# lorenlugosch/end-to-end-SLU

Hardware: AMD Instinct MI355X
Metric: utterances/sec (train step, 3 s @16 kHz, B=64) (higher is better)
Workload: dtype f32 (trainable stages: exact fp32 MFMA; convolutions and GRU contractions of FROZEN stages: bf16x3 = every fp32 operand split EXACTLY into 3 bf16 terms (3 x 8 = 24 significand bits, fp32's exponent range), 6 bf16 MFMA products per fp32 product (only terms below 2^-24 |a b| dropped), fp32 accumulatio; 1 GPU; experiments/no_unfreezing.cfg SLU train step (frozen SincNet/conv/biGRU encoder in train mode + intent biGRU trained): fwd + 3-slot CE + bwd + grad all-reduce + Adam; batch_per_gpu=64, global_batch=64, samples_per_utterance=48000, parallelism=dp1, encoder_lookahead_batches=20

## Files before the change

### end-to-end-slu_amd/csrc/slu_gru_bf16.hip

```cpp
#include "slu_bf16.h"
#include <type_traits>

namespace slu {

__device__ __forceinline__ float bf_sigmoid(float x) {
  return __builtin_amdgcn_rcpf(1.0f + __builtin_amdgcn_exp2f(-1.4426950408889634f * x));
}
__device__ __forceinline__ float bf_tanh(float x) {
  return 1.0f - 2.0f * __builtin_amdgcn_rcpf(1.0f + __builtin_amdgcn_exp2f(2.8853900817779268f * x));
}

__device__ __forceinline__ void lds_barrier() { asm volatile("s_waitcnt lgkmcnt(0)\n\ts_barrier" ::: "memory"); }

__device__ __forceinline__ float mul_rnd(float a, float b) {
#pragma clang fp contract(off)
  return a * b;
}
__device__ __forceinline__ float add_rnd(float a, float b) {
#pragma clang fp contract(off)
  return a + b;
}

struct GruBfParams {
  const float* gx;
  const unsigned short* xp; long long x_plane;
  const uint4* wih; const float* b_ih;
  const float* w_hh[2];
  const float* b_hh[2];
  float* out;
  float* reserve;
  unsigned short* planes; long long plane;
  const unsigned* keep;
  float keep_scale;
  int T, B, D;
};

template <int H, int NS, int KI, int EPI>
struct GruLds {
  static constexpr int ROWB = H * 2;
  static constexpr int GXROW = 3 * H + 8;
  static constexpr int OROW = H + 4;
  static constexpr int PROWB = H * 2 + 16;
  static constexpr int HBUF = 2 * NS * 16 * ROWB;
  static constexpr int BIAS = KI > 0 ? 2 * 3 * H * 4 : 0;
  static constexpr int GXS = KI > 0 ? 0 : 2 * 16 * GXROW * 4;
  static constexpr int OST = EPI == 1 ? 2 * NS * 16 * PROWB : 2 * 16 * OROW * 4;
  static constexpr int BYTES = HBUF + BIAS + GXS + OST;
};

template <int H, int NS, int KI, int EPI, bool REV>
__device__ __forceinline__ void gru_bf_fwd_body(const GruBfParams& p) {
  constexpr int NW = H / 16;
  constexpr int KC = H / 32;
  constexpr int SLOTS = H / 8;
  constexpr bool BIAS_LDS = KI > 0;
  typedef Split<NS> SP;
  typedef GruLds<H, NS, KI, EPI> LD;
  constexpr int ROWB = LD::ROWB, GXROW = LD::GXROW, OROW = LD::OROW, PROWB = LD::PROWB;
  extern __shared__ __attribute__((aligned(16))) unsigned char smem[];
  unsigned char* const hbuf = smem;
  float* const bias_s = reinterpret_cast<float*>(smem + LD::HBUF);
  float* const gxs = reinterpret_cast<float*>(smem + LD::HBUF + LD::BIAS);
  unsigned char* const ost = smem + LD::HBUF + LD::BIAS + LD::GXS;
  const int tid = threadIdx.x, lane = tid & 63;
  const int w = __builtin_amdgcn_readfirstlane(tid >> 6);
  const int i = lane & 15, kg = lane >> 4;
  constexpr int dir = REV ? 1 : 0;
  const int b0 = blockIdx.x * 16;
  const int u0 = w * 16 + kg * 4;
  const int T = p.T, B = p.B, D = p.D;
  const int seq = b0 + i;
  const int seqc = seq < B ? seq : B - 1;

  if constexpr (NS == 2) f16_denorm_flush();

  uint4 wb[3][KC][NS];
  {
    const float* __restrict__ W = p.w_hh[dir];
#pragma unroll
    for (int g = 0; g < 3; ++g)
#pragma unroll
      for (int c = 0; c < KC; ++c) {
        const float* src = W + (size_t)(g * H + w * 16 + i) * H + c * 32 + kg * 8;
        const float4 lo = *reinterpret_cast<const float4*>(src), hi = *reinterpret_cast<const float4*>(src + 4);
        const float v[8] = {lo.x, lo.y, lo.z, lo.w, hi.x, hi.y, hi.z, hi.w};
        unsigned short s[8][NS];
#pragma unroll
        for (int e = 0; e < 8; ++e) split_terms<NS>(v[e], s[e]);
#pragma unroll
        for (int pl = 0; pl < NS; ++pl) {
          uint4 o;
          o.x = s[0][pl] | ((unsigned)s[1][pl] << 16); o.y = s[2][pl] | ((unsigned)s[3][pl] << 16);
          o.z = s[4][pl] | ((unsigned)s[5][pl] << 16); o.w = s[6][pl] | ((unsigned)s[7][pl] << 16);
          wb[g][c][pl] = o;
        }
      }
  }
  float bh[3][4];
  if constexpr (BIAS_LDS) {
    for (int x = tid; x < 3 * H; x += H * 4) {
      bias_s[x] = p.b_hh[dir][x];
      bias_s[3 * H + x] = p.b_ih[(size_t)dir * 3 * H + x];
    }
  } else {
#pragma unroll
    for (int g = 0; g < 3; ++g) {
      const float4 v = *reinterpret_cast<const float4*>(p.b_hh[dir] + g * H + u0);
      bh[g][0] = v.x; bh[g][1] = v.y; bh[g][2] = v.z; bh[g][3] = v.w;
    }
  }
  constexpr int KIA = KI > 0 ? KI : 1;
  uint4 wi[3][KIA][NS];
  if constexpr (KI > 0) {
    const int NTI = p.D * 3 * NW;
#pragma unroll
    for (int g = 0; g < 3; ++g)
#pragma unroll
      for (int c = 0; c < KI; ++c)
#pragma unroll
        for (int pl = 0; pl < NS; ++pl)
          wi[g][c][pl] = p.wih[(size_t)pl * KI * NTI * 64 + ((size_t)c * NTI + dir * 3 * NW + g * NW + w) * 64 + lane];
  }
  auto xproj = [&](const uint4 (&xa)[KIA][NS], float (&o)[3][4]) {
    f32x4 ax[SP::NACC][3];
#pragma unroll
    for (int a = 0; a < SP::NACC; ++a)
#pragma unroll
      for (int g = 0; g < 3; ++g) ax[a][g] = f32x4{0.f, 0.f, 0.f, 0.f};
#pragma unroll
    for (int c = 0; c < KIA; ++c)
#pragma unroll
      for (int q = 0; q < SP::NPAIR; ++q)
#pragma unroll
        for (int g = 0; g < 3; ++g)
          ax[SP::ACC(q)][g] = mfma_split<NS>(wi[g][c][SP::PB(q)], xa[c][SP::PA(q)], ax[SP::ACC(q)][g]);
#pragma unroll
    for (int g = 0; g < 3; ++g) {
      const f32x4 v = split_result<NS>(ax[0][g], ax[SP::NACC - 1][g]);
      const float4 bi = *reinterpret_cast<const float4*>(&bias_s[BIAS_LDS ? 3 * H + g * H + u0 : 0]);
      o[g][0] = v[0] + bi.x; o[g][1] = v[1] + bi.y; o[g][2] = v[2] + bi.z; o[g][3] = v[3] + bi.w;
    }
  };
  auto xload = [&](int t_, uint4 (&xa)[KIA][NS]) {
    const unsigned short* base = p.xp + ((size_t)t_ * B + seqc) * (32 * KIA) + kg * 8;
#pragma unroll
    for (int c = 0; c < KIA; ++c)
#pragma unroll
      for (int pl = 0; pl < NS; ++pl)
        xa[c][pl] = *reinterpret_cast<const uint4*>(base + (size_t)pl * p.x_plane + c * 32);
  };

  constexpr int RW = 16 / NW;
  constexpr int GLR = 3 * H / 4;
  auto gx_g = [&](int j) { const int f = j * 64 + lane; return min(b0 + RW * w + f / GLR, B - 1) * D * 3 * H + dir * 3 * H + (f % GLR) * 4; };
  auto gx_s = [&](int j) { const int f = j * 64 + lane; return (RW * w + f / GLR) * GXROW + (f % GLR) * 4; };
  const int gx_g0 = gx_g(0), gx_g1 = gx_g(1), gx_g2 = gx_g(2);
  const int gx_s0 = gx_s(0), gx_s1 = gx_s(1), gx_s2 = gx_s(2);
  const size_t gx_ts = (size_t)B * D * 3 * H, out_ts = (size_t)B * D * H;
#define SLU_GX_REQUEST(t_, a, b, c)                                                         \
  do {                                                                                      \
    const float* gp__ = p.gx + (size_t)(t_) * gx_ts;                                        \
    a = *reinterpret_cast<const float4*>(gp__ + gx_g0);                                     \
    b = *reinterpret_cast<const float4*>(gp__ + gx_g1);                                     \
    c = *reinterpret_cast<const float4*>(gp__ + gx_g2);                                     \
  } while (0)
#define SLU_GX_STAGE(buf, a, b, c)                                                          \
  do {                                                                                      \
    float* gs__ = gxs + (buf) * (16 * GXROW);                                               \
    *reinterpret_cast<float4*>(gs__ + gx_s0) = a;                                           \
    *reinterpret_cast<float4*>(gs__ + gx_s1) = b;                                           \
    *reinterpret_cast<float4*>(gs__ + gx_s2) = c;                                           \
  } while (0)
  const int orow = RW * w + lane / (H / 4), oc16 = lane % (H / 4);
  const bool orow_ok = b0 + orow < B;
  const int o_goff = (b0 + orow) * D * H + dir * H + oc16 * 4;

  int a_off[KC];
#pragma unroll
  for (int c = 0; c < KC; ++c) a_off[c] = i * ROWB + (((c * 4 + kg) ^ i) & (SLOTS - 1)) * 16;
  const int h_off = i * ROWB + ((((u0 >> 3) ^ i) & (SLOTS - 1)) * 16) + (u0 & 7) * 2;
  const int gs_off = i * GXROW + u0;
  const int os_off = i * OROW + u0;
  const int ps_off = i * PROWB + u0 * 2;
  const int kw_off = seqc * ((D * H) >> 5) + ((dir * H + u0) >> 5);
  const int kw_sh = (dir * H + u0) & 31;
  const size_t kw_ts = (size_t)B * ((D * H) >> 5);
  const bool drop = EPI > 0 && p.keep != nullptr;

  for (int x = tid; x < 2 * NS * 16 * ROWB / 4; x += H * 4) reinterpret_cast<unsigned*>(hbuf)[x] = 0u;
  float hprev[4] = {0.f, 0.f, 0.f, 0.f};
  float gcur[3][4];
  unsigned kcur = 0;
  {
    const int t0 = dir ? T - 1 : 0;
    if constexpr (KI > 0) {
      __syncthreads();
      uint4 xa0[KIA][NS];
      xload(t0, xa0);
      xproj(xa0, gcur);
    } else {
      float4 ga, gb, gc;
      SLU_GX_REQUEST(t0, ga, gb, gc);
      SLU_GX_STAGE(0, ga, gb, gc);
    }
    if (drop) kcur = p.keep[(size_t)t0 * kw_ts + kw_off];
  }
  float held[4] = {0.f, 0.f, 0.f, 0.f};
  int pend_t = -1;
  int pend_buf = 0;
  auto flush = [&]() {
    if (pend_t < 0) return;
    if constexpr (EPI == 1) {
      constexpr int LPR = H / 8;
      constexpr int NCH = NS * 16 * LPR / 64;
      for (int c = w; c < NCH; c += NW) {
        const int f = c * 64 + lane, pl = f / (16 * LPR), r = (f / LPR) % 16, c16 = f % LPR;
        if (b0 + r < B) {
          const uint4 v = *reinterpret_cast<const uint4*>(ost + ((pend_buf * NS + pl) * 16 + r) * PROWB + c16 * 16);
          *reinterpret_cast<uint4*>(p.planes + (size_t)pl * p.plane + (size_t)pend_t * out_ts + (b0 + r) * D * H + dir * H + c16 * 8) = v;
        }
      }
    } else {
      if (orow_ok) {
        const float4 v = *reinterpret_cast<const float4*>(reinterpret_cast<const float*>(ost) + (pend_buf * 16 + orow) * OROW + oc16 * 4);
        *reinterpret_cast<float4*>(p.out + (size_t)pend_t * out_ts + o_goff) = v;
      }
    }
  };
  __syncthreads();
  __builtin_amdgcn_s_waitcnt(0x0F70);

  auto step = [&](auto cur_c, const int s) {
    constexpr int cur = decltype(cur_c)::value;
    const int t = dir ? T - 1 - s : s;
    const int tn = (s + 1 < T) ? (dir ? t - 1 : t + 1) : t;

    if constexpr (BIAS_LDS) {
#pragma unroll
      for (int g = 0; g < 3; ++g) {
        const float4 v = *reinterpret_cast<const float4*>(&bias_s[g * H + u0]);
        bh[g][0] = v.x; bh[g][1] = v.y; bh[g][2] = v.z; bh[g][3] = v.w;
      }
    }
    if constexpr (KI == 0) {
#pragma unroll
      for (int g = 0; g < 3; ++g) {
        const float4 v = *reinterpret_cast<const float4*>(gxs + cur * (16 * GXROW) + gs_off + g * H);
        gcur[g][0] = v.x; gcur[g][1] = v.y; gcur[g][2] = v.z; gcur[g][3] = v.w;
      }
    }
    f32x4 accs[SP::NACC][3];
#pragma unroll
    for (int a = 0; a < SP::NACC; ++a)
#pragma unroll
      for (int g = 0; g < 3; ++g) accs[a][g] = f32x4{0.f, 0.f, 0.f, 0.f};
    float gn[4];
#pragma unroll
    for (int r = 0; r < 4; ++r) {
      accs[0][0][r] = gcur[0][r] + bh[0][r];
      accs[0][1][r] = gcur[1][r] + bh[1][r];
      accs[0][2][r] = bh[2][r];
      gn[r] = gcur[2][r];
    }
    const unsigned kbits = kcur >> kw_sh;

    float gnext[3][4];
    float4 gl0 = make_float4(0.f, 0.f, 0.f, 0.f), gl1 = gl0, gl2 = gl0;
    uint4 xan[KIA][NS];
    if constexpr (KI > 0) xload(tn, xan);
    else SLU_GX_REQUEST(tn, gl0, gl1, gl2);
    unsigned knext = 0;
    if (drop) knext = p.keep[(size_t)tn * kw_ts + kw_off];
    flush();

    const unsigned char* hc = hbuf + cur * (NS * 16 * ROWB);
    float hn[4];
#pragma unroll
    for (int c = 0; c < KC; ++c) {
      uint4 fa[NS];
#pragma unroll
      for (int pl = 0; pl < NS; ++pl) fa[pl] = *reinterpret_cast<const uint4*>(hc + pl * (16 * ROWB) + a_off[c]);
#pragma unroll
      for (int q = 0; q < SP::NPAIR; ++q)
#pragma unroll
        for (int g = 0; g < 3; ++g)
          accs[SP::ACC(q)][g] = mfma_split<NS>(wb[g][c][SP::PB(q)], fa[SP::PA(q)], accs[SP::ACC(q)][g]);
    }
    f32x4 acc[3];
#pragma unroll
    for (int g = 0; g < 3; ++g) acc[g] = split_result<NS>(accs[0][g], accs[SP::NACC - 1][g]);

#pragma unroll
    for (int r = 0; r < 4; ++r) {
      const float rr = bf_sigmoid(acc[0][r]);
      const float zz = bf_sigmoid(acc[1][r]);
      const float nn = bf_tanh(gn[r] + rr * acc[2][r]);
      hn[r] = nn + zz * (hprev[r] - nn);
    }
    {
      unsigned char* __restrict__ hnext = hbuf + (cur ^ 1) * (NS * 16 * ROWB);
      if constexpr (NS == 2) {
        unsigned hi01, lo01, hi23, lo23;
        split_f16x2_pair_flush(hn[0], hn[1], hi01, lo01);
        split_f16x2_pair_flush(hn[2], hn[3], hi23, lo23);
        *reinterpret_cast<uint2*>(hnext + h_off) = make_uint2(hi01, hi23);
        *reinterpret_cast<uint2*>(hnext + 16 * ROWB + h_off) = make_uint2(lo01, lo23);
      } else if constexpr (NS == 3) {
        unsigned w01[3], w23[3];
        split_bf16x3_pair(hn[0], hn[1], w01);
        split_bf16x3_pair(hn[2], hn[3], w23);
#pragma unroll
        for (int pl = 0; pl < 3; ++pl)
          *reinterpret_cast<uint2*>(hnext + pl * (16 * ROWB) + h_off) = make_uint2(w01[pl], w23[pl]);
      } else {
        unsigned short sp[4][NS];
#pragma unroll
        for (int r = 0; r < 4; ++r) split_terms<NS>(hn[r], sp[r]);
#pragma unroll
        for (int pl = 0; pl < NS; ++pl)
          *reinterpret_cast<uint2*>(hnext + pl * (16 * ROWB) + h_off) =
              make_uint2(sp[0][pl] | ((unsigned)sp[1][pl] << 16), sp[2][pl] | ((unsigned)sp[3][pl] << 16));
      }
    }
    if constexpr (EPI == 0) {
      *reinterpret_cast<float4*>(reinterpret_cast<float*>(ost) + cur * (16 * OROW) + os_off) = make_float4(hn[0], hn[1], hn[2], hn[3]);
      pend_t = t; pend_buf = cur;
    } else {
      float m[4];
#pragma unroll
      for (int r = 0; r < 4; ++r)
        m[r] = drop ? mul_rnd(hn[r], ((kbits >> r) & 1u) ? p.keep_scale : 0.0f) : hn[r];
      const bool even = dir ? (t & 1) == 0 : cur == 0;
      const bool single = even && t == T - 1;
      const bool emit = dir ? even : (!even || single);
      pend_t = -1;
      if (!emit) {
#pragma unroll
        for (int r = 0; r < 4; ++r) held[r] = dir ? m[r] : add_rnd(0.0f, m[r]);
      } else {
        float v[4];
#pragma unroll
        for (int r = 0; r < 4; ++r) {
          const float first = dir ? add_rnd(0.0f, m[r]) : held[r];
          const float second = dir ? held[r] : m[r];
          v[r] = mul_rnd(add_rnd(first, second), 0.5f);
        }
        if (single) {
          asm volatile("" ::: "memory");
#pragma unroll
          for (int r = 0; r < 4; ++r) v[r] = add_rnd(0.0f, m[r]);
        }
        pend_t = t >> 1; pend_buf = cur;
        if constexpr (EPI == 2) {
          *reinterpret_cast<float4*>(reinterpret_cast<float*>(ost) + cur * (16 * OROW) + os_off) = make_float4(v[0], v[1], v[2], v[3]);
        } else if constexpr (NS == 2) {
          unsigned hi01, lo01, hi23, lo23;
          split_f16x2_pair_flush(v[0], v[1], hi01, lo01);
          split_f16x2_pair_flush(v[2], v[3], hi23, lo23);
          *reinterpret_cast<uint2*>(ost + ((cur * NS + 0) * 16) * PROWB + ps_off) = make_uint2(hi01, hi23);
          *reinterpret_cast<uint2*>(ost + ((cur * NS + 1) * 16) * PROWB + ps_off) = make_uint2(lo01, lo23);
        } else if constexpr (NS == 3) {
          unsigned w01[3], w23[3];
          split_bf16x3_pair(v[0], v[1], w01);
          split_bf16x3_pair(v[2], v[3], w23);
#pragma unroll
          for (int pl = 0; pl < 3; ++pl)
            *reinterpret_cast<uint2*>(ost + ((cur * NS + pl) * 16) * PROWB + ps_off) = make_uint2(w01[pl], w23[pl]);
        } else {
          unsigned short sp[4][NS];
#pragma unroll
          for (int r = 0; r < 4; ++r) split_terms<NS>(v[r], sp[r]);
#pragma unroll
          for (int pl = 0; pl < NS; ++pl)
            *reinterpret_cast<uint2*>(ost + ((cur * NS + pl) * 16) * PROWB + ps_off) =
                make_uint2(sp[0][pl] | ((unsigned)sp[1][pl] << 16), sp[2][pl] | ((unsigned)sp[3][pl] << 16));
        }
      }
    }
    if constexpr (KI > 0) {
      xproj(xan, gnext);
#pragma unroll
      for (int g = 0; g < 3; ++g)
#pragma unroll
        for (int r = 0; r < 4; ++r) gcur[g][r] = gnext[g][r];
    } else {
      SLU_GX_STAGE(cur ^ 1, gl0, gl1, gl2);
    }
#pragma unroll
    for (int r = 0; r < 4; ++r) hprev[r] = hn[r];
    kcur = knext;
    lds_barrier();
  };
  {
    int s = 0;
    for (; s + 1 < T; s += 2) {
      step(std::integral_constant<int, 0>{}, s);
      step(std::integral_constant<int, 1>{}, s + 1);
    }
    if (s < T) step(std::integral_constant<int, 0>{}, s);
  }
  flush();
#undef SLU_GX_REQUEST
#undef SLU_GX_STAGE
}

template <int H, int NS, int KI, int EPI>
__global__ void __launch_bounds__(H * 4)
gru_bf_fwd_kernel(const GruBfParams p) {
  if (blockIdx.y) gru_bf_fwd_body<H, NS, KI, EPI, true>(p);
  else gru_bf_fwd_body<H, NS, KI, EPI, false>(p);
}

template <int H, int NS, int EPI>
struct Gru2Lds {
  static constexpr int ROWB = H * 2;
  static constexpr int OROW = H + 4;
  static constexpr int PROWB = H * 2 + 16;
  static constexpr int HB = NS * 16 * ROWB;
  static constexpr int GXB = 16 * 3 * H * 4;
  static constexpr int KBB = 16 * (H / 32) * 4;
  static constexpr int OSB = EPI == 1 ? NS * 16 * PROWB : 16 * OROW * 4;
  static constexpr int HBUF = 0;
  static constexpr int GXR = HBUF + 2 * HB;
  static constexpr int KBR = GXR + 3 * GXB;
  static constexpr int BIAS = KBR + 3 * KBB;
  static constexpr int OST = BIAS + 3 * H * 4;
  static constexpr int HP = OST + 2 * OSB;
  static constexpr int HELD = HP + 2 * 16 * H * 4;
  static constexpr int BYTES = HELD + (EPI > 0 ? 2 * 16 * H * 4 : 0);
};

__device__ __forceinline__ void dma_b128(const void* base, unsigned voff, unsigned lds_addr) {
  asm volatile("s_mov_b32 m0, %2\n\ts_nop 0\n\tglobal_load_lds_dwordx4 %0, %1" :: "v"(voff), "s"(base), "s"(lds_addr) : "memory");
}
__device__ __forceinline__ void dma_b32(const void* base, unsigned voff, unsigned lds_addr) {
  asm volatile("s_mov_b32 m0, %2\n\ts_nop 0\n\tglobal_load_lds_dword %0, %1" :: "v"(voff), "s"(base), "s"(lds_addr) : "memory");
}

template <int H, int NS, int EPI>
__global__ void __launch_bounds__(H * 4)
gru_bf2_fwd_kernel(const GruBfParams p) {
  static_assert(H == 128, "two-tile recurrence: H = 128 (8 waves = two per SIMD, one keep-word DMA per chunk)");
  constexpr int NW = H / 16, KC = H / 32, SLOTS = H / 8;
  typedef Split<NS> SP;
  typedef Gru2Lds<H, NS, EPI> LD;
  constexpr int ROWB = LD::ROWB, OROW = LD::OROW, PROWB = LD::PROWB;
  constexpr int PCS = 3 * H / 4;
  extern __shared__ __attribute__((aligned(16))) unsigned char smem[];
  typedef __attribute__((address_space(3))) void* lptr_t;
  const unsigned lds0 = (unsigned)(size_t)(lptr_t)smem;
  float* const bias_s = reinterpret_cast<float*>(smem + LD::BIAS);
  const int tid = threadIdx.x, lane = tid & 63;
  const int w = __builtin_amdgcn_readfirstlane(tid >> 6);
  const int i = lane & 15, kg = lane >> 4;
  const int dir = blockIdx.y;
  const int b0 = blockIdx.x * 32;
  const int u0 = w * 16 + kg * 4;
  const int T = p.T, B = p.B, D = p.D;

  if constexpr (NS == 2) f16_denorm_flush();

  uint4 wb[3][KC][NS];
  {
    const float* __restrict__ W = p.w_hh[dir];
#pragma unroll
    for (int g = 0; g < 3; ++g)
#pragma unroll
      for (int c = 0; c < KC; ++c) {
        const float* src = W + (size_t)(g * H + w * 16 + i) * H + c * 32 + kg * 8;
        const float4 lo = *reinterpret_cast<const float4*>(src), hi = *reinterpret_cast<const float4*>(src + 4);
        const float v[8] = {lo.x, lo.y, lo.z, lo.w, hi.x, hi.y, hi.z, hi.w};
        unsigned short s[8][NS];
#pragma unroll
        for (int e = 0; e < 8; ++e) split_terms<NS>(v[e], s[e]);
#pragma unroll
        for (int pl = 0; pl < NS; ++pl) {
          uint4 o;
          o.x = s[0][pl] | ((unsigned)s[1][pl] << 16); o.y = s[2][pl] | ((unsigned)s[3][pl] << 16);
          o.z = s[4][pl] | ((unsigned)s[5][pl] << 16); o.w = s[6][pl] | ((unsigned)s[7][pl] << 16);
          wb[g][c][pl] = o;
        }
      }
  }
  for (int x = tid; x < 3 * H; x += H * 4) bias_s[x] = p.b_hh[dir][x];
  for (int x = tid; x < 2 * LD::HB / 4; x += H * 4) reinterpret_cast<unsigned*>(smem + LD::HBUF)[x] = 0u;
  __syncthreads();

  const bool drop = EPI > 0 && p.keep != nullptr;
  unsigned gv[2][3];
#pragma unroll
  for (int x = 0; x < 2; ++x)
#pragma unroll
    for (int j = 0; j < 3; ++j) {
      const int P = (3 * w + j) * 64 + lane, row = P / PCS, q = P % PCS;
      gv[x][j] = (unsigned)((min(b0 + 16 * x + row, B - 1) * D * 3 * H + dir * 3 * H) * 4 + (q ^ (row & 15)) * 16);
    }
  unsigned kv[2];
  const int KW = (D * H) >> 5;
#pragma unroll
  for (int x = 0; x < 2; ++x)
    kv[x] = drop ? (unsigned)((min(b0 + 16 * x + (lane >> 2), B - 1) * KW + dir * (H >> 5) + (lane & 3)) * 4) : (unsigned)(lane * 4);
  const void* const kbase = drop ? (const void*)p.keep : (const void*)p.gx;
  const size_t gx_ts = (size_t)B * D * 3 * H * 4, kw_ts = drop ? (size_t)B * KW * 4 : 0, out_ts = (size_t)B * D * H;
  const unsigned gx_m0 = lds0 + LD::GXR + 3 * w * 1024, kb_m0 = lds0 + LD::KBR;
  auto dma_chunk = [&](int x, int t_, int slot) {
    const char* gb = reinterpret_cast<const char*>(p.gx) + (size_t)t_ * gx_ts;
    const unsigned m = gx_m0 + slot * LD::GXB;
    const unsigned v0 = x ? gv[1][0] : gv[0][0], v1 = x ? gv[1][1] : gv[0][1], v2 = x ? gv[1][2] : gv[0][2];
    dma_b128(gb, v0, m);
    dma_b128(gb, v1, m + 1024);
    dma_b128(gb, v2, m + 2048);
    dma_b32(reinterpret_cast<const char*>(kbase) + (size_t)t_ * kw_ts, x ? kv[1] : kv[0], kb_m0 + slot * LD::KBB);
  };

  const int a_off0 = i * ROWB + ((kg ^ i) & (SLOTS - 1)) * 16;
  const int h_off = i * ROWB + ((((u0 >> 3) ^ i) & (SLOTS - 1)) * 16) + (u0 & 7) * 2;
  const int gs_off0 = (i * PCS + ((u0 >> 2) ^ i)) * 16;
  const int hp_off = (i * H + u0) * 4;
  const int kb_off = (i * (H >> 5) + (u0 >> 5)) * 4;
  const int kb_sh = u0 & 31;
  const int os_off = i * OROW + u0;
  const int ps_off = i * PROWB + u0 * 2;
  const int orow = (16 / NW) * w + lane / (H / 4), oc16 = lane % (H / 4);

  f32x4 accs[2][SP::NACC][3];
  float gn[2][4];
  unsigned kb[2] = {0u, 0u};
  int pend[2] = {-1, -1};
#pragma unroll
  for (int x = 0; x < 2; ++x) {
#pragma unroll
    for (int r = 0; r < 4; ++r) gn[x][r] = 0.f;
    *reinterpret_cast<float4*>(smem + LD::HP + x * (16 * H * 4) + hp_off) = make_float4(0.f, 0.f, 0.f, 0.f);
    if constexpr (EPI > 0) *reinterpret_cast<float4*>(smem + LD::HELD + x * (16 * H * 4) + hp_off) = make_float4(0.f, 0.f, 0.f, 0.f);
  }
#pragma unroll
  for (int x = 0; x < 2; ++x)
#pragma unroll
    for (int a = 0; a < SP::NACC; ++a)
#pragma unroll
      for (int g = 0; g < 3; ++g) accs[x][a][g] = f32x4{0.f, 0.f, 0.f, 0.f};

#define SLU_G2_M(X, slot)                                                                                              \
// ... 147 lines not shown
  dma_chunk(0, tt(0), 0);
  dma_chunk(1, tt(0), 1);
  asm volatile("s_waitcnt vmcnt(0)" ::: "memory");
  __syncthreads();

  int sl = 0;
  SLU_G2_PHASE(0, true, false, 0, tt(1));
  for (int s = 0; s + 1 < T; ++s) {
    SLU_G2_PHASE(1, true, true, tt(s), tt(s + 1));
    SLU_G2_PHASE(0, true, true, tt(s), tt(s + 2));
  }
  SLU_G2_PHASE(1, true, true, tt(T - 1), tt(T - 1));
  SLU_G2_PHASE(0, false, true, tt(T - 1), tt(T - 1));
  SLU_G2_FLUSH(1);
  asm volatile("s_waitcnt vmcnt(0)" ::: "memory");
#undef SLU_G2_PHASE
#undef SLU_G2_FLUSH
#undef SLU_G2_G
#undef SLU_G2_M
}

template <int H, int NS>
__global__ void __launch_bounds__(H * 4)
gru_bf_fwd_rs_kernel(const GruBfParams p) {
  constexpr int NW = H / 16, KC = H / 32, ROWB = H * 2, SLOTS = H / 8;
  typedef Split<NS> SP;
  __shared__ __attribute__((aligned(16))) unsigned char hbuf[2][NS][16 * ROWB];
  const int tid = threadIdx.x, lane = tid & 63;
  const int w = __builtin_amdgcn_readfirstlane(tid >> 6);
  const int i = lane & 15, kg = lane >> 4;
  const int dir = blockIdx.y;
  const int b0 = blockIdx.x * 16;
  const int j = w * 16 + i;
  const int T = p.T, B = p.B, D = p.D;

  uint4 wb[3][KC][NS];
  {
    const float* __restrict__ W = p.w_hh[dir];
#pragma unroll
    for (int g = 0; g < 3; ++g)
#pragma unroll
      for (int c = 0; c < KC; ++c) {
        const float* src = W + (size_t)(g * H + j) * H + c * 32 + kg * 8;
        const float4 lo = *reinterpret_cast<const float4*>(src), hi = *reinterpret_cast<const float4*>(src + 4);
        const float v[8] = {lo.x, lo.y, lo.z, lo.w, hi.x, hi.y, hi.z, hi.w};
        unsigned short s[8][NS];
#pragma unroll
        for (int e = 0; e < 8; ++e) split_terms<NS>(v[e], s[e]);
#pragma unroll
        for (int pl = 0; pl < NS; ++pl) {
          uint4 o;
          o.x = s[0][pl] | ((unsigned)s[1][pl] << 16); o.y = s[2][pl] | ((unsigned)s[3][pl] << 16);
          o.z = s[4][pl] | ((unsigned)s[5][pl] << 16); o.w = s[6][pl] | ((unsigned)s[7][pl] << 16);
          wb[g][c][pl] = o;
        }
      }
  }
  const float bhr = p.b_hh[dir][j], bhz = p.b_hh[dir][H + j], bhn = p.b_hh[dir][2 * H + j];
  for (int x = tid; x < 2 * NS * 16 * ROWB / 4; x += H * 4) reinterpret_cast<unsigned*>(&hbuf[0][0][0])[x] = 0u;
  float hprev[4] = {0.f, 0.f, 0.f, 0.f};
  int g_off[4], o_off[4];
#pragma unroll
  for (int r = 0; r < 4; ++r) {
    const int b = b0 + 4 * kg + r;
    g_off[r] = (b < B ? b : 0) * D * 3 * H;
    o_off[r] = b < B ? b * D * H : -1;
  }
  const size_t gx_ts = (size_t)B * D * 3 * H, out_ts = (size_t)B * D * H;
  const float* __restrict__ gxd = p.gx + (size_t)dir * 3 * H + j;
  float* __restrict__ outd = p.out + (size_t)dir * H + j;
  int a_off[KC];
#pragma unroll
  for (int c = 0; c < KC; ++c) a_off[c] = i * ROWB + (((c * 4 + kg) ^ i) & (SLOTS - 1)) * 16;
  int h_off[4];
#pragma unroll
  for (int r = 0; r < 4; ++r) {
    const int row = 4 * kg + r;
    h_off[r] = row * ROWB + ((((j >> 3) ^ row) & (SLOTS - 1)) * 16) + (j & 7) * 2;
  }
  float gr[4], gz[4], gn[4];
  {
    const int t0 = dir ? T - 1 : 0;
#pragma unroll
    for (int r = 0; r < 4; ++r) {
      const float* g = gxd + (size_t)t0 * gx_ts + g_off[r];
      gr[r] = g[0]; gz[r] = g[H]; gn[r] = g[2 * H];
    }
  }
  __syncthreads();

  for (int s = 0; s < T; ++s) {
    const int t = dir ? T - 1 - s : s;
    const int cur = s & 1;
    float ngr[4], ngz[4], ngn[4];
    const int tn = (s + 1 < T) ? (dir ? t - 1 : t + 1) : t;
#pragma unroll
    for (int r = 0; r < 4; ++r) {
      const float* g = gxd + (size_t)tn * gx_ts + g_off[r];
      ngr[r] = g[0]; ngz[r] = g[H]; ngn[r] = g[2 * H];
    }
    f32x4 accs[SP::NACC][3];
#pragma unroll
    for (int a = 0; a < SP::NACC; ++a)
#pragma unroll
      for (int g = 0; g < 3; ++g) accs[a][g] = f32x4{0.f, 0.f, 0.f, 0.f};
#pragma unroll
    for (int c = 0; c < KC; ++c) {
      uint4 fa[NS];
#pragma unroll
      for (int pl = 0; pl < NS; ++pl) fa[pl] = *reinterpret_cast<const uint4*>(&hbuf[cur][pl][a_off[c]]);
#pragma unroll
      for (int q = 0; q < SP::NPAIR; ++q)
#pragma unroll
        for (int g = 0; g < 3; ++g)
          accs[SP::ACC(q)][g] = mfma_split<NS>(fa[SP::PA(q)], wb[g][c][SP::PB(q)], accs[SP::ACC(q)][g]);
    }
    f32x4 acc[3];
#pragma unroll
    for (int g = 0; g < 3; ++g) acc[g] = split_result<NS>(accs[0][g], accs[SP::NACC - 1][g]);

    float hn[4], rr[4], zz[4], nn[4], qq[4];
#pragma unroll
    for (int r = 0; r < 4; ++r) {
      rr[r] = bf_sigmoid(gr[r] + (acc[0][r] + bhr));
      zz[r] = bf_sigmoid(gz[r] + (acc[1][r] + bhz));
      qq[r] = acc[2][r] + bhn;
      nn[r] = bf_tanh(gn[r] + rr[r] * qq[r]);
      hn[r] = (1.0f - zz[r]) * nn[r] + zz[r] * hprev[r];
    }
    {
      float4* __restrict__ rs = reinterpret_cast<float4*>(
          p.reserve + ((((size_t)dir * T + t) * gridDim.x + blockIdx.x) * NW + w) * (5 * 256)) + lane;
      rs[0 * 64] = make_float4(rr[0], rr[1], rr[2], rr[3]);
      rs[1 * 64] = make_float4(zz[0], zz[1], zz[2], zz[3]);
      rs[2 * 64] = make_float4(nn[0], nn[1], nn[2], nn[3]);
      rs[3 * 64] = make_float4(qq[0], qq[1], qq[2], qq[3]);
      rs[4 * 64] = make_float4(hprev[0], hprev[1], hprev[2], hprev[3]);
    }
    unsigned char* __restrict__ hnext = &hbuf[cur ^ 1][0][0];
#pragma unroll
    for (int r = 0; r < 4; ++r) {
      unsigned short sp[NS];
      split_terms<NS>(hn[r], sp);
#pragma unroll
      for (int pl = 0; pl < NS; ++pl) *reinterpret_cast<unsigned short*>(hnext + pl * (16 * ROWB) + h_off[r]) = sp[pl];
      if (o_off[r] >= 0) outd[(size_t)t * out_ts + o_off[r]] = hn[r];
    }
#pragma unroll
    for (int r = 0; r < 4; ++r) { hprev[r] = hn[r]; gr[r] = ngr[r]; gz[r] = ngz[r]; gn[r] = ngn[r]; }
    __syncthreads();
  }
}

template <int H, int NS, int KI, int EPI>
static void gru_bf_launch(dim3 grid, hipStream_t st, const GruBfParams& p) {
  constexpr int lds = GruLds<H, NS, KI, EPI>::BYTES;
  static bool raised = false;
  if (lds > 64 * 1024 && !raised) {
    (void)hipFuncSetAttribute((const void*)gru_bf_fwd_kernel<H, NS, KI, EPI>, hipFuncAttributeMaxDynamicSharedMemorySize, lds);
    raised = true;
  }
  hipLaunchKernelGGL((gru_bf_fwd_kernel<H, NS, KI, EPI>), grid, dim3(H * 4), lds, st, p);
}

template <int H, int NS, int EPI>
static void gru_bf2_launch(hipStream_t st, const GruBfParams& p) {
  constexpr int lds = Gru2Lds<H, NS, EPI>::BYTES;
  static bool raised = false;
  if (lds > 64 * 1024 && !raised) {
    (void)hipFuncSetAttribute((const void*)gru_bf2_fwd_kernel<H, NS, EPI>, hipFuncAttributeMaxDynamicSharedMemorySize, lds);
    raised = true;
  }
  hipLaunchKernelGGL((gru_bf2_fwd_kernel<H, NS, EPI>), dim3((unsigned)cdiv(p.B, 32), (unsigned)p.D), dim3(H * 4), lds, st, p);
}

template <int H, int EPI>
static int gru_bf_dispatch(int nsplit, int ki, int seq_tiles, dim3 grid, hipStream_t st, const GruBfParams& p) {
  if (seq_tiles == 2) {
    if constexpr (H == 128) {
      if (nsplit == 3) gru_bf2_launch<128, 3, EPI>(st, p);
      else if (nsplit == 2) gru_bf2_launch<128, 2, EPI>(st, p);
      else gru_bf2_launch<128, 1, EPI>(st, p);
    }
    SLU_CHECK_LAUNCH("gru_bf2_fwd_kernel");
    return SLU_OK;
  }
  if (ki > 0) {
    if constexpr (H == 128) {
      if (nsplit == 3) {
        if (ki == 1) gru_bf_launch<128, 3, 1, EPI>(grid, st, p); else gru_bf_launch<128, 3, 2, EPI>(grid, st, p);
      } else {
        if (ki == 1) gru_bf_launch<128, 2, 1, EPI>(grid, st, p); else gru_bf_launch<128, 2, 2, EPI>(grid, st, p);
      }
    }
  } else if (nsplit == 3) {
    gru_bf_launch<H, 3, 0, EPI>(grid, st, p);
  } else if (nsplit == 2) {
    gru_bf_launch<H, 2, 0, EPI>(grid, st, p);
  } else {
    gru_bf_launch<H, 1, 0, EPI>(grid, st, p);
  }
  SLU_CHECK_LAUNCH("gru_bf_fwd_kernel");
  return SLU_OK;
}

}

using namespace slu;

static int gru_bf_common(const char* who, GruBfParams& p, const float* gx, const float* w_hh_fwd, const float* w_hh_rev,
                         const float* b_hh_fwd, const float* b_hh_rev, const void* x_planes, int64_t x_plane_stride,
                         int64_t K, const void* w_ih_packed, const float* b_ih, int64_t T, int64_t B, int64_t H, int64_t D,
                         int nsplit, bool has_reserve, int seq_tiles) {
  SLU_REQUIRE((gx || x_planes) && w_hh_fwd && b_hh_fwd, "%s: null pointer", who);
  SLU_REQUIRE(seq_tiles >= 0 && seq_tiles <= 2, "%s: seq_tiles must be 0 / 1 (one 16-sequence tile per workgroup) or 2", who);
  if (seq_tiles == 2 && !(H == 128 && gx && !x_planes && !has_reserve && B * D * 3 * H < (1LL << 30)))
    SLU_FAIL(SLU_ERR_UNSUPPORTED, "%s: two sequence tiles per workgroup are instantiated for H = 128, gx input (no fused "
             "projection), no reserve, B * D * 3H < 2^30 (got H %lld, B %lld)", who, (long long)H, (long long)B);
  const bool fused = x_planes != nullptr;
  if (fused) {
    SLU_REQUIRE(!gx && w_ih_packed && b_ih && !has_reserve, "%s: the fused input projection takes x_planes, "
                "w_ih_packed and b_ih instead of gx, and no reserve (frozen layers only)", who);
    if (!((nsplit == 2 || nsplit == 3) && H == 128 && K >= 1 && K <= 64))
      SLU_FAIL(SLU_ERR_UNSUPPORTED, "%s: the fused input projection is instantiated for f16x2 / bf16x3 (nsplit 2 / 3), "
               "H = 128 and at most 64 input channels (got nsplit %d, H %lld, K %lld)", who, nsplit, (long long)H, (long long)K);
    SLU_REQUIRE(x_plane_stride >= T * B * (cdiv(K, 32) * 32) && ((uintptr_t)x_planes & 15) == 0 && (x_plane_stride & 7) == 0,
                "%s: x plane stride / alignment", who);
  }
  SLU_REQUIRE(D == 1 || (D == 2 && w_hh_rev && b_hh_rev), "%s: D must be 1 or 2 (with reverse weights)", who);
  SLU_REQUIRE(T > 0 && B > 0, "%s: non-positive T or B", who);
  SLU_REQUIRE(nsplit >= 1 && nsplit <= 3, "%s: nsplit must be 1 (bf16), 2 (f16x2) or 3 (bf16x3)", who);
  if (H != 64 && H != 128)
    SLU_FAIL(SLU_ERR_UNSUPPORTED, "%s: hidden size %lld not instantiated (64, 128)", who, (long long)H);
  SLU_REQUIRE(cdiv(B, 16) <= 65535 && B * D * 3 * H < (1LL << 31), "%s: B too large", who);
  SLU_REQUIRE(!gx || ((uintptr_t)gx & 15) == 0, "%s: gx must be 16-byte aligned", who);
  SLU_REQUIRE(((uintptr_t)b_hh_fwd & 15) == 0 && ((uintptr_t)b_hh_rev & 15) == 0, "%s: biases must be 16-byte aligned", who);
  p.xp = (const unsigned short*)x_planes; p.x_plane = x_plane_stride; p.wih = (const uint4*)w_ih_packed; p.b_ih = b_ih;
  p.gx = gx; p.w_hh[0] = w_hh_fwd; p.w_hh[1] = w_hh_rev; p.b_hh[0] = b_hh_fwd; p.b_hh[1] = b_hh_rev;
  p.out = nullptr; p.reserve = nullptr; p.planes = nullptr; p.plane = 0; p.keep = nullptr; p.keep_scale = 1.0f;
  p.T = (int)T; p.B = (int)B; p.D = (int)D;
  return SLU_OK;
}

extern "C" int slu_gru_seq_fwd_bf16(const float* gx, const float* w_hh_fwd, const float* w_hh_rev,
                                    const float* b_hh_fwd, const float* b_hh_rev, float* out, float* reserve,
                                    const void* x_planes, int64_t x_plane_stride, int64_t K, const void* w_ih_packed,
                                    const float* b_ih, int64_t T, int64_t B, int64_t H, int64_t D, int nsplit,
                                    int seq_tiles, void* stream) {
  SLU_REQUIRE(out, "slu_gru_seq_fwd_bf16: null pointer");
  GruBfParams p;
  int rc = gru_bf_common("slu_gru_seq_fwd_bf16", p, gx, w_hh_fwd, w_hh_rev, b_hh_fwd, b_hh_rev, x_planes, x_plane_stride, K,
                         w_ih_packed, b_ih, T, B, H, D, nsplit, reserve != nullptr, seq_tiles);
  if (rc) return rc;
  p.out = out; p.reserve = reserve;
  dim3 grid((unsigned)cdiv(B, 16), (unsigned)D);
  hipStream_t st = (hipStream_t)stream;
  if (reserve) {
#define SLU_RS(H_, NS_) hipLaunchKernelGGL((gru_bf_fwd_rs_kernel<H_, NS_>), grid, dim3(H_ * 4), 0, st, p)
    if (H == 128) { if (nsplit == 3) SLU_RS(128, 3); else if (nsplit == 2) SLU_RS(128, 2); else SLU_RS(128, 1); }
    else { if (nsplit == 3) SLU_RS(64, 3); else if (nsplit == 2) SLU_RS(64, 2); else SLU_RS(64, 1); }
#undef SLU_RS
    SLU_CHECK_LAUNCH("gru_bf_fwd_rs_kernel");
    return SLU_OK;
  }
  SLU_REQUIRE(((uintptr_t)out & 15) == 0, "slu_gru_seq_fwd_bf16: out must be 16-byte aligned");
  const int ki = x_planes ? (K <= 32 ? 1 : 2) : 0;
  return H == 128 ? gru_bf_dispatch<128, 0>(nsplit, ki, seq_tiles, grid, st, p) : gru_bf_dispatch<64, 0>(nsplit, ki, seq_tiles, grid, st, p);
}

extern "C" int slu_gru_seq_fwd_pool_bf16(const float* gx, const float* w_hh_fwd, const float* w_hh_rev,
                                         const float* b_hh_fwd, const float* b_hh_rev, float* out_pooled,
                                         void* out_planes, int64_t out_plane_stride, const uint32_t* keep_bits, float p_drop,
                                         const void* x_planes, int64_t x_plane_stride, int64_t K, const void* w_ih_packed,
                                         const float* b_ih, int64_t T, int64_t B, int64_t H, int64_t D, int nsplit,
                                         int seq_tiles, void* stream) {
  SLU_REQUIRE((out_pooled != nullptr) != (out_planes != nullptr),
              "slu_gru_seq_fwd_pool_bf16: exactly one of out_pooled and out_planes");
  SLU_REQUIRE(p_drop >= 0.0f && p_drop < 1.0f && (keep_bits || p_drop == 0.0f),
              "slu_gru_seq_fwd_pool_bf16: dropout p in [0, 1), with keep_bits when p > 0");
  GruBfParams p;
  int rc = gru_bf_common("slu_gru_seq_fwd_pool_bf16", p, gx, w_hh_fwd, w_hh_rev, b_hh_fwd, b_hh_rev, x_planes,
                         x_plane_stride, K, w_ih_packed, b_ih, T, B, H, D, nsplit, false, seq_tiles);
  if (rc) return rc;
  if ((D * H) % 32 != 0)
    SLU_FAIL(SLU_ERR_UNSUPPORTED, "slu_gru_seq_fwd_pool_bf16: D * H must be a multiple of 32 (got %lld)", (long long)(D * H));
  const int64_t T_out = cdiv(T, 2);
  if (out_planes)
    SLU_REQUIRE(out_plane_stride >= T_out * B * D * H && ((uintptr_t)out_planes & 7) == 0 && (out_plane_stride & 3) == 0,
                "slu_gru_seq_fwd_pool_bf16: plane stride / alignment");
  else
    SLU_REQUIRE(((uintptr_t)out_pooled & 15) == 0, "slu_gru_seq_fwd_pool_bf16: out_pooled must be 16-byte aligned");
  p.out = out_pooled; p.planes = (unsigned short*)out_planes; p.plane = out_plane_stride;
  p.keep = p_drop > 0.0f ? keep_bits : nullptr; p.keep_scale = 1.0f / (1.0f - p_drop);
  dim3 grid((unsigned)cdiv(B, 16), (unsigned)D);
  hipStream_t st = (hipStream_t)stream;
  const int ki = x_planes ? (K <= 32 ? 1 : 2) : 0;
  if (out_planes)
    return H == 128 ? gru_bf_dispatch<128, 1>(nsplit, ki, seq_tiles, grid, st, p) : gru_bf_dispatch<64, 1>(nsplit, ki, seq_tiles, grid, st, p);
  return H == 128 ? gru_bf_dispatch<128, 2>(nsplit, ki, seq_tiles, grid, st, p) : gru_bf_dispatch<64, 2>(nsplit, ki, seq_tiles, grid, st, p);
}
```

Baseline: 372,300 utterances/s.

## Stage GRU input tiles via async global-to-LDS DMA and spill input weights to LDS

For the fused bf16x3 input-projection GRU path, the per-step x tile loads now use global_load_lds_dwordx4 into a double-buffered LDS area, prefetched two steps ahead, in place of per-thread register loads. Part of the input-weight fragments move from registers into a large LDS region (up to 160 KB), which relieves VGPR pressure. The output staging buffer is single-buffered with an extra barrier to make room. Per-device LDS-limit raising is also made atomic. The cost is higher LDS usage, extra waitcnt and barriers, and LDS reads of weights on every step.

```diff
diff --git a/end-to-end-slu_amd/csrc/slu_gru_bf16.hip b/end-to-end-slu_amd/csrc/slu_gru_bf16.hip
--- a/end-to-end-slu_amd/csrc/slu_gru_bf16.hip
+++ b/end-to-end-slu_amd/csrc/slu_gru_bf16.hip
@@ -1,4 +1,5 @@
 #include "slu_bf16.h"
+#include <atomic>
 #include <type_traits>
 
 namespace slu {
@@ -11,6 +12,12 @@
 }
 
 __device__ __forceinline__ void lds_barrier() { asm volatile("s_waitcnt lgkmcnt(0)\n\ts_barrier" ::: "memory"); }
+
+__device__ __forceinline__ void glds_b128(const void* base, unsigned voff, unsigned lds_addr) {
+  unsigned keep;
+  asm volatile("s_mov_b32 %0, m0\n\ts_mov_b32 m0, %3\n\ts_nop 0\n\tglobal_load_lds_dwordx4 %1, %2\n\ts_mov_b32 m0, %0"
+               : "=&s"(keep) : "v"(voff), "s"(base), "s"(lds_addr) : "memory");
+}
 
 __device__ __forceinline__ float mul_rnd(float a, float b) {
 #pragma clang fp contract(off)
@@ -44,8 +51,22 @@
   static constexpr int HBUF = 2 * NS * 16 * ROWB;
   static constexpr int BIAS = KI > 0 ? 2 * 3 * H * 4 : 0;
   static constexpr int GXS = KI > 0 ? 0 : 2 * 16 * GXROW * 4;
-  static constexpr int OST = EPI == 1 ? 2 * NS * 16 * PROWB : 2 * 16 * OROW * 4;
-  static constexpr int BYTES = HBUF + BIAS + GXS + OST;
+  static constexpr bool FUSED3 = KI > 0 && NS == 3;
+  static constexpr int NOST = FUSED3 && EPI > 0 ? 1 : 2;
+  static constexpr int OST = NOST * (EPI == 1 ? NS * 16 * PROWB : 16 * OROW * 4);
+  static constexpr int XS1 = NS * KI * 64 * 16;
+  static constexpr int XST = FUSED3 ? 2 * XS1 : 0;
+  static constexpr int WSLOT = (H / 16) * 64 * 16;
+  static constexpr int BASE = HBUF + BIAS + GXS + OST + XST;
+  static constexpr int WFIT = (160 * 1024 - BASE) / WSLOT;
+  static constexpr int WMAX = KI > 1 ? 14 : 6;
+  static constexpr int WSLOTS = FUSED3 ? (WFIT < WMAX ? WFIT : WMAX) : 0;
+  static constexpr int BYTES = BASE + WSLOTS * WSLOT;
+  static __device__ __host__ constexpr int wslot(int g, int c, int pl) {
+    if (!FUSED3) return -1;
+    const int x = (2 - pl) * 3 * KI + c * 3 + g;
+    return x < WSLOTS ? x : -1;
+  }
 };
 
 template <int H, int NS, int KI, int EPI, bool REV>
@@ -62,6 +83,9 @@
   float* const bias_s = reinterpret_cast<float*>(smem + LD::HBUF);
   float* const gxs = reinterpret_cast<float*>(smem + LD::HBUF + LD::BIAS);
   unsigned char* const ost = smem + LD::HBUF + LD::BIAS + LD::GXS;
+  uint4* const xs = reinterpret_cast<uint4*>(smem + LD::HBUF + LD::BIAS + LD::GXS + LD::OST);
+  uint4* const wis = reinterpret_cast<uint4*>(smem + LD::BASE);
+  constexpr bool FUSED3 = LD::FUSED3;
   const int tid = threadIdx.x, lane = tid & 63;
   const int w = __builtin_amdgcn_readfirstlane(tid >> 6);
   const int i = lane & 15, kg = lane >> 4;
@@ -118,9 +142,16 @@
 #pragma unroll
       for (int c = 0; c < KI; ++c)
 #pragma unroll
-        for (int pl = 0; pl < NS; ++pl)
-          wi[g][c][pl] = p.wih[(size_t)pl * KI * NTI * 64 + ((size_t)c * NTI + dir * 3 * NW + g * NW + w) * 64 + lane];
-  }
+        for (int pl = 0; pl < NS; ++pl) {
+          const uint4 v = p.wih[(size_t)pl * KI * NTI * 64 + ((size_t)c * NTI + dir * 3 * NW + g * NW + w) * 64 + lane];
+          if (LD::wslot(g, c, pl) >= 0) wis[(LD::wslot(g, c, pl) * NW + w) * 64 + lane] = v;
+          else wi[g][c][pl] = v;
+        }
+  }
+  auto wfrag = [&](int g, int c, int pl) -> uint4 {
+    if (LD::wslot(g, c, pl) >= 0) return wis[(LD::wslot(g, c, pl) * NW + w) * 64 + lane];
+    return wi[g][c][pl];
+  };
   auto xproj = [&](const uint4 (&xa)[KIA][NS], float (&o)[3][4]) {
     f32x4 ax[SP::NACC][3];
 #pragma unroll
@@ -133,7 +164,7 @@
       for (int q = 0; q < SP::NPAIR; ++q)
 #pragma unroll
         for (int g = 0; g < 3; ++g)
-          ax[SP::ACC(q)][g] = mfma_split<NS>(wi[g][c][SP::PB(q)], xa[c][SP::PA(q)], ax[SP::ACC(q)][g]);
+          ax[SP::ACC(q)][g] = mfma_split<NS>(wfrag(g, c, SP::PB(q)), xa[c][SP::PA(q)], ax[SP::ACC(q)][g]);
 #pragma unroll
     for (int g = 0; g < 3; ++g) {
       const f32x4 v = split_result<NS>(ax[0][g], ax[SP::NACC - 1][g]);
@@ -148,6 +179,21 @@
 #pragma unroll
       for (int pl = 0; pl < NS; ++pl)
         xa[c][pl] = *reinterpret_cast<const uint4*>(base + (size_t)pl * p.x_plane + c * 32);
+  };
+  constexpr int NX = NS * KIA * 64;
+  const bool x_ld = FUSED3 && w < NS * KIA;
+  const unsigned x_voff = ((unsigned)seqc * (32 * KIA) + (w % KIA) * 32 + kg * 8) * 2;
+  typedef __attribute__((address_space(3))) void* lptr_t;
+  const unsigned xs_addr = (unsigned)(size_t)(lptr_t)xs + w * 1024;
+  auto t_of = [&](int s_) { s_ = min(s_, T - 1); return dir ? T - 1 - s_ : s_; };
+  auto xdma = [&](int t_, int buf) {
+    glds_b128(p.xp + (size_t)(w / KIA) * p.x_plane + (size_t)t_ * B * (32 * KIA), x_voff, xs_addr + buf * (NX * 16));
+  };
+  auto xfrag = [&](int buf, uint4 (&xa)[KIA][NS]) {
+#pragma unroll
+    for (int c = 0; c < KIA; ++c)
+#pragma unroll
+      for (int pl = 0; pl < NS; ++pl) xa[c][pl] = xs[buf * (NS * KIA * 64) + (pl * KIA + c) * 64 + lane];
   };
 
   constexpr int RW = 16 / NW;
@@ -196,7 +242,14 @@
     if constexpr (KI > 0) {
       __syncthreads();
       uint4 xa0[KIA][NS];
-      xload(t0, xa0);
+      if constexpr (FUSED3) {
+        if (x_ld) { xdma(t_of(0), 0); xdma(t_of(1), 1); }
+        asm volatile("s_waitcnt vmcnt(0)" ::: "memory");
+        __syncthreads();
+        xfrag(0, xa0);
+      } else {
+        xload(t0, xa0);
+      }
       xproj(xa0, gcur);
     } else {
       float4 ga, gb, gc;
@@ -234,6 +287,7 @@
     constexpr int cur = decltype(cur_c)::value;
     const int t = dir ? T - 1 - s : s;
     const int tn = (s + 1 < T) ? (dir ? t - 1 : t + 1) : t;
+    constexpr int ob = LD::NOST == 2 ? cur : 0;
 
     if constexpr (BIAS_LDS) {
 #pragma unroll
@@ -267,7 +321,8 @@
     float gnext[3][4];
     float4 gl0 = make_float4(0.f, 0.f, 0.f, 0.f), gl1 = gl0, gl2 = gl0;
     uint4 xan[KIA][NS];
-    if constexpr (KI > 0) xload(tn, xan);
+    if constexpr (FUSED3) { if (x_ld) xdma(t_of(s + 2), cur); }
+    else if constexpr (KI > 0) xload(tn, xan);
     else SLU_GX_REQUEST(tn, gl0, gl1, gl2);
     unsigned knext = 0;
     if (drop) knext = p.keep[(size_t)tn * kw_ts + kw_off];
@@ -323,8 +378,8 @@
       }
     }
     if constexpr (EPI == 0) {
-      *reinterpret_cast<float4*>(reinterpret_cast<float*>(ost) + cur * (16 * OROW) + os_off) = make_float4(hn[0], hn[1], hn[2], hn[3]);
-      pend_t = t; pend_buf = cur;
+      *reinterpret_cast<float4*>(reinterpret_cast<float*>(ost) + ob * (16 * OROW) + os_off) = make_float4(hn[0], hn[1], hn[2], hn[3]);
+      pend_t = t; pend_buf = ob;
     } else {
       float m[4];
 #pragma unroll
@@ -337,6 +392,7 @@
       if (!emit) {
 #pragma unroll
         for (int r = 0; r < 4; ++r) held[r] = dir ? m[r] : add_rnd(0.0f, m[r]);
+        if constexpr (FUSED3) asm volatile("");
       } else {
         float v[4];
 #pragma unroll
@@ -349,35 +405,37 @@
           asm volatile("" ::: "memory");
 #pragma unroll
           for (int r = 0; r < 4; ++r) v[r] = add_rnd(0.0f, m[r]);
+          if constexpr (LD::NOST == 1) lds_barrier();
         }
-        pend_t = t >> 1; pend_buf = cur;
+        pend_t = t >> 1; pend_buf = ob;
         if constexpr (EPI == 2) {
-          *reinterpret_cast<float4*>(reinterpret_cast<float*>(ost) + cur * (16 * OROW) + os_off) = make_float4(v[0], v[1], v[2], v[3]);
+          *reinterpret_cast<float4*>(reinterpret_cast<float*>(ost) + ob * (16 * OROW) + os_off) = make_float4(v[0], v[1], v[2], v[3]);
         } else if constexpr (NS == 2) {
           unsigned hi01, lo01, hi23, lo23;
           split_f16x2_pair_flush(v[0], v[1], hi01, lo01);
           split_f16x2_pair_flush(v[2], v[3], hi23, lo23);
-          *reinterpret_cast<uint2*>(ost + ((cur * NS + 0) * 16) * PROWB + ps_off) = make_uint2(hi01, hi23);
-          *reinterpret_cast<uint2*>(ost + ((cur * NS + 1) * 16) * PROWB + ps_off) = make_uint2(lo01, lo23);
+          *reinterpret_cast<uint2*>(ost + ((ob * NS + 0) * 16) * PROWB + ps_off) = make_uint2(hi01, hi23);
+          *reinterpret_cast<uint2*>(ost + ((ob * NS + 1) * 16) * PROWB + ps_off) = make_uint2(lo01, lo23);
         } else if constexpr (NS == 3) {
           unsigned w01[3], w23[3];
           split_bf16x3_pair(v[0], v[1], w01);
           split_bf16x3_pair(v[2], v[3], w23);
 #pragma unroll
           for (int pl = 0; pl < 3; ++pl)
-            *reinterpret_cast<uint2*>(ost + ((cur * NS + pl) * 16) * PROWB + ps_off) = make_uint2(w01[pl], w23[pl]);
+            *reinterpret_cast<uint2*>(ost + ((ob * NS + pl) * 16) * PROWB + ps_off) = make_uint2(w01[pl], w23[pl]);
         } else {
           unsigned short sp[4][NS];
 #pragma unroll
           for (int r = 0; r < 4; ++r) split_terms<NS>(v[r], sp[r]);
 #pragma unroll
           for (int pl = 0; pl < NS; ++pl)
-            *reinterpret_cast<uint2*>(ost + ((cur * NS + pl) * 16) * PROWB + ps_off) =
+            *reinterpret_cast<uint2*>(ost + ((ob * NS + pl) * 16) * PROWB + ps_off) =
                 make_uint2(sp[0][pl] | ((unsigned)sp[1][pl] << 16), sp[2][pl] | ((unsigned)sp[3][pl] << 16));
         }
       }
     }
     if constexpr (KI > 0) {
+      if constexpr (FUSED3) xfrag(cur ^ 1, xan);
       xproj(xan, gnext);
 #pragma unroll
       for (int g = 0; g < 3; ++g)
@@ -389,6 +447,7 @@
 #pragma unroll
     for (int r = 0; r < 4; ++r) hprev[r] = hn[r];
     kcur = knext;
+    if constexpr (FUSED3) asm volatile("s_waitcnt vmcnt(0)" ::: "memory");
     lds_barrier();
   };
   {
@@ -842,25 +901,29 @@
   }
 }
 
+template <void (*KERNEL)(const GruBfParams)>
+static bool lds_limit_raise(int lds) {
+  constexpr int MAX_DEV = 64;
+  static std::atomic<bool> raised[MAX_DEV];
+  int dev = -1;
+  const bool known = hipGetDevice(&dev) == hipSuccess && dev >= 0 && dev < MAX_DEV;
+  if (known && raised[dev].load(std::memory_order_acquire)) return true;
+  if (hipFuncSetAttribute((const void*)KERNEL, hipFuncAttributeMaxDynamicSharedMemorySize, lds) != hipSuccess) return false;
+  if (known) raised[dev].store(true, std::memory_order_release);
+  return true;
+}
+
 template <int H, int NS, int KI, int EPI>
 static void gru_bf_launch(dim3 grid, hipStream_t st, const GruBfParams& p) {
   constexpr int lds = GruLds<H, NS, KI, EPI>::BYTES;
-  static bool raised = false;
-  if (lds > 64 * 1024 && !raised) {
-    (void)hipFuncSetAttribute((const void*)gru_bf_fwd_kernel<H, NS, KI, EPI>, hipFuncAttributeMaxDynamicSharedMemorySize, lds);
-    raised = true;
-  }
+  if (lds > 64 * 1024 && !lds_limit_raise<gru_bf_fwd_kernel<H, NS, KI, EPI>>(lds)) return;
   hipLaunchKernelGGL((gru_bf_fwd_kernel<H, NS, KI, EPI>), grid, dim3(H * 4), lds, st, p);
 }
 
 template <int H, int NS, int EPI>
 static void gru_bf2_launch(hipStream_t st, const GruBfParams& p) {
   constexpr int lds = Gru2Lds<H, NS, EPI>::BYTES;
-  static bool raised = false;
-  if (lds > 64 * 1024 && !raised) {
-    (void)hipFuncSetAttribute((const void*)gru_bf2_fwd_kernel<H, NS, EPI>, hipFuncAttributeMaxDynamicSharedMemorySize, lds);
-    raised = true;
-  }
+  if (lds > 64 * 1024 && !lds_limit_raise<gru_bf2_fwd_kernel<H, NS, EPI>>(lds)) return;
   hipLaunchKernelGGL((gru_bf2_fwd_kernel<H, NS, EPI>), dim3((unsigned)cdiv(p.B, 32), (unsigned)p.D), dim3(H * 4), lds, st, p);
 }
 
```

Result: no change. 376,500 utterances/s, median of 2 (+1.1%).
